# neuraloperator/graph-pde

Hardware: NVIDIA H100
Metric: NNConv edge-applications/s (higher is better)
Workload: dtype f16

## Files before the change

graph_pde_b200/csrc/api.cu:

```cuda
#include <cstdarg>
#include <cstdio>
#include <cstdlib>
#include <cstring>
#include <new>
#include <vector>

#include "common.cuh"
#include "kernels.h"
#include "options.h"

namespace nnc {

namespace {
thread_local char g_err[512] = "";
}

void set_error(const char* fmt, ...) {
  va_list ap;
  va_start(ap, fmt);
  vsnprintf(g_err, sizeof(g_err), fmt, ap);
  va_end(ap);
}

namespace {
// ... 315 lines not shown
  return launch_gemm_tc(W->prec, h, P->E, 0, static_cast<int>(P->E), W->Kp, W->W3n, NK, W->B3, 0, Kmat, NK, st, nullptr, 0, 0,
                        0, nullptr, nullptr, 0, 0, hpad);
}

int apply_edge(const Plan* P, const Weights* W, const void* Kmat, const float* x, const float* root, const float* bias,
               int aggr_mean, float* out, cudaStream_t st, unsigned node_flags) {
  NNC_REQUIRE(!(node_flags & NNCONV_APPLY_RESIDUAL) || W->cin == W->cout, NNCONV_ERR_ARG,
              "NNCONV_APPLY_RESIDUAL needs in_channels == out_channels");
  int s = launch_out_init(x, root, bias, P->N, W->cin, W->cout, out, st, node_flags);
  if (s) return s;
  if (P->E == 0 || P->n_src == 0) return NNCONV_OK;
  return launch_apply_edge(W->prec, P, W, Kmat, x, aggr_mean, out, st, node_flags);
}

struct ApplyLayout {
  size_t off_Xc, off_cvec, off_xs, off_flags, off_Y, fixed_bytes, per_node;
};
constexpr int kMaxPipeBatches = 1 << 14;

static ApplyLayout layout_apply(const Plan* P, const Weights* W) {
  Carver c(nullptr, ~size_t(0));
  ApplyLayout L{};
  const size_t S = P->n_src > 0 ? P->n_src : 1;
  L.off_Xc = c.off; c.take<char>((S + 128) * W->cin_p * W->esize * (W->split ? 3 : 1));
  L.off_cvec = c.off; c.take<float>(S * W->cout);
  L.off_xs = c.off; c.take<float>(S);
  L.off_flags = c.off; c.take<int>(5 * kMaxPipeBatches);
  L.off_Y = c.off;
  L.fixed_bytes = c.off;
  L.per_node = static_cast<size_t>(W->cout) * W->Kp * W->esize * (W->split ? 2 : 1);
  return L;
}

size_t apply_ws_bytes(const Plan* P, const Weights* W, size_t want_y_bytes) {
  ApplyLayout L = layout_apply(P, W);
  size_t nodes = want_y_bytes / L.per_node;
  if (nodes < 1) nodes = 1;
  if (nodes > static_cast<size_t>(P->n_src > 0 ? P->n_src : 1)) nodes = P->n_src > 0 ? P->n_src : 1;
  return L.fixed_bytes + nodes * L.per_node + 1024;
}

static bool fused_geometry(const Weights* W, int64_t n_src, int64_t nodes_cap, int* ring_out, int64_t* nb_out) {
  const Options& opt = options();
  const bool no_fuse_env = opt.no_fuse != 0 && !W->split;
  if (W->prec == PREC_FP32 || no_fuse_env || !apply_fused_supported(W)) return false;
  int ring = opt.ring;
  if (opt.ring_deep && nodes_cap / 128 > ring) ring = nodes_cap / 128 < 16 ? static_cast<int>(nodes_cap / 128) : 16;
  if (nodes_cap < ring) ring = nodes_cap >= 2 ? static_cast<int>(nodes_cap) : 1;
  int64_t nb = nodes_cap / ring;
  if (nb >= 128) nb = nb / 128 * 128;
  if (nb > n_src) nb = n_src;
  *ring_out = ring;
  *nb_out = nb;
  return ring >= 2;
}

int apply(const Plan* P, const Weights* W, const void* h, const float* x, const float* root, const float* bias,
          int aggr_mean, float* out, void* ws, size_t ws_bytes, cudaStream_t st, int64_t* launches, unsigned node_flags) {
  int s;
  NNC_REQUIRE(!(node_flags & NNCONV_APPLY_RESIDUAL) || W->cin == W->cout, NNCONV_ERR_ARG,
              "NNCONV_APPLY_RESIDUAL needs in_channels == out_channels");
  if (P->E == 0 || P->n_src == 0) {
    ProfScope ps(PK_NODE_PREP, st);
    s = launch_out_init(x, root, bias, P->N, W->cin, W->cout, out, st, node_flags);
    if (s == NNCONV_OK && launches) ++*launches;
    return s;
  }
  const bool tc = tc_shapes_supported(W);
// ... 103 lines not shown
  };
  auto launch_c = [&](int64_t b) -> int {
    const int64_t c0 = b * nb_max;
    const int nb = static_cast<int>((P->n_src - c0) < nb_max ? (P->n_src - c0) : nb_max);
    const int tb = h_tile_ptr[c0], te = h_tile_ptr[c0 + nb];
    PipeFlags pf{};
    pf.pdl = pipe;
    pf.wait_ok = pipe ? okY + b : nullptr;
    pf.done_cnt = pipe ? cntC + b : nullptr;
    pf.done_ok = pipe ? okC + b : nullptr;
    if (pipe && b == n_batches - 1) {
      pf.join_ok = okC;
      pf.join_n = static_cast<int>(n_batches - 1);
    }
    ProfScope ps(PK_CONV, st);
    return launch_conv_tc(W->prec, P, h, W->Kp, Ybuf[b % 3], nb, W->cout, tb, te, static_cast<int>(c0), cvec, xs,
                          aggr_mean, out, st, pipe ? &pf : nullptr);
  };
  s = launch_y(0);
  if (s) return s;
  for (int64_t b = 0; b < n_batches; ++b) {
    if (b + 1 < n_batches) {
      s = launch_y(b + 1);
      if (s) return s;
    }
    s = launch_c(b);
    if (s) return s;
  }
  if (launches) *launches += 2 * n_batches;
  return NNCONV_OK;
}

constexpr int64_t kUnitEdges = 2 * kTileEdges;
constexpr size_t kStreamYBytes = size_t(48) << 20;

static size_t h_row_bytes(const Weights* W) { return static_cast<size_t>(W->Kp) * 2 * (W->split ? 2 : 1); }

static int src_of_edge(const Plan* P, int64_t e) {
  const int* g = P->h_group_ptr;
  int lo = 0, hi = P->n_src;
  while (hi - lo > 1) {
    const int mid = (lo + hi) / 2;
    if (g[mid] <= e) lo = mid; else hi = mid;
  }
  return lo;
}

static int64_t unit_floor(const Plan* P, int64_t lim) {
  if (lim >= P->E) return P->E;
  if (lim <= 0) return 0;
  const int c = src_of_edge(P, lim);
  const int64_t g = P->h_group_ptr[c];
  return g + (lim - g) / kUnitEdges * kUnitEdges;
}

bool is_unit_boundary(const Plan* P, int64_t e) { return e >= 0 && e <= P->E && unit_floor(P, e) == e; }

static UnitRange edge_range(const Plan* P, int64_t e_lo, int64_t e_hi) {
  UnitRange r;
  const int c_lo = src_of_edge(P, e_lo);
  r.u_begin = P->h_unit_ptr[c_lo] + static_cast<int>((e_lo - P->h_group_ptr[c_lo]) / kUnitEdges);
  if (e_hi >= P->E) {
    r.u_end = P->n_units;
  } else {
    const int c_hi = src_of_edge(P, e_hi);
    r.u_end = P->h_unit_ptr[c_hi] + static_cast<int>((e_hi - P->h_group_ptr[c_hi]) / kUnitEdges);
  }
  r.c_begin = c_lo;
  r.c_end = src_of_edge(P, e_hi - 1) + 1;
  r.e_base = e_lo;
  r.h_rows = round_up64(e_hi - e_lo, 128);
  return r;
}

static int tile_at(const Plan* P, int64_t e) {
  if (e >= P->E) return P->n_tiles;
  const int c = src_of_edge(P, e);
  return P->h_tile_ptr[c] + static_cast<int>((e - P->h_group_ptr[c]) / kTileEdges);
}

struct StreamLayout {
  size_t off_apply, apply_bytes, off_h, off_ef, ef_bytes;
  int64_t rows;
};

static StreamLayout layout_stream(const Plan* P, const Weights* W, size_t ws_bytes) {
  StreamLayout L{};
  L.off_apply = kEfHeader;
  L.apply_bytes = round_up64(static_cast<int64_t>(apply_ws_bytes(P, W, kStreamYBytes)), 1024);
  L.off_h = L.off_apply + L.apply_bytes;
  const size_t fixed = L.off_h + 4096;
  const size_t row = h_row_bytes(W) + ef_row_bytes(W);
  L.rows = ws_bytes > fixed ? static_cast<int64_t>((ws_bytes - fixed) / row / 128 * 128) : 0;
  L.off_ef = L.off_h + static_cast<size_t>(L.rows) * h_row_bytes(W);
  L.ef_bytes = static_cast<size_t>(L.rows) * ef_row_bytes(W) + 4096;
  return L;
}

static int64_t count_chunks(const Plan* P, int64_t E_res, int64_t rows) {
  int64_t n = 0;
  for (int64_t e = E_res; e < P->E; e = unit_floor(P, e + rows)) ++n;
  return n;
}

int stream_split(const Plan* P, const Weights* W, size_t resident_bytes, size_t chunk_ws_bytes, int64_t* E_res,
                 size_t* h_res_bytes, size_t* ws_bytes, int64_t* n_chunks) {
  NNC_REQUIRE(W->prec == PREC_F16 || W->prec == PREC_BF16 || W->prec == PREC_F16X2, NNCONV_ERR_UNSUPPORTED,
              "streamed edge features need precision f16, bf16 or f16x2");
  const size_t hrow = h_row_bytes(W);
  const size_t full = static_cast<size_t>(round_up64(P->E, 128)) * hrow;
  *E_res = resident_bytes >= full ? P->E : unit_floor(P, static_cast<int64_t>(resident_bytes / hrow) / 128 * 128);
  *h_res_bytes = static_cast<size_t>(round_up64(*E_res, 128)) * hrow;
  const size_t row = hrow + ef_row_bytes(W);
  int64_t rows = static_cast<int64_t>(chunk_ws_bytes / row) / 128 * 128;
  const int64_t rest = round_up64(P->E - *E_res, 128);
  if (rows > rest) rows = rest;
  if (rows < kUnitEdges) rows = kUnitEdges;
  StreamLayout L = layout_stream(P, W, 0);
  *ws_bytes = L.off_h + 4096 + static_cast<size_t>(rows) * row;
  *n_chunks = count_chunks(P, *E_res, rows);
  return NNCONV_OK;
}
// ... 599 lines not shown
```

graph_pde_b200/csrc/apply_tc.cu:

```cuda
#include <type_traits>

#include "kernels.h"
#include "options.h"
#include "tc05.cuh"
#include "tmap.h"

namespace nnc {

int tc_num_sms();

namespace {

using namespace tc05;

constexpr int kMaxSlots = 16;
constexpr int kMaxAStages = 10;
constexpr int kTU = 2;
constexpr int kATileBytes = 128 * 64 * 2;
constexpr int kYStages = 2;
constexpr int kThreads = 14 * 32;
constexpr int kConvProducer = 12, kYProducer = 13;
constexpr int kQueue = 8;
constexpr int kScatterPitch = 272;
constexpr int kScatterBytes = 8 * 32 * kScatterPitch;
constexpr int kYScratchBytes = 4 * acc_scratch_bytes<16>();

struct ApplyArgs {
  const int* tile_c;
  const int* tile_e0;
  const int* tile_cnt;
  const int* tile_ptr;
  const int* unit_ptr;
  const int* unit_t;
  const int* unit_u;
  const int* dst_sorted;
  const float* inv_deg;
  const float* cvec;
  const float* xs;
  float* out;
  int u_begin, u_end, c_begin, c_end, e_base;
  int nb, n_batches, ring;
  int nb_slots, passes, a_stages, e_pad;
  int split_nk;
  int Kp;
  const float* y_scale;
  int NY;
  int num_kx;
  void* Yring;
  int* cntY;
  int* okY;
  int* cntC;
  int* okC;
  int* cntU;
  unsigned long long y_store_policy;
  unsigned long long a_policy;
  int scatter_mode;
  int debug_scatter;
  TraceBuf trace;
};

struct HMaps {
  CUtensorMap m[8];
};

__device__ __forceinline__ void raise_when_all(int* cnt, int* ok, int target) {
  const int prev = atomicAdd(cnt, 1);
  if (prev == target - 1) {
    __threadfence();
    asm volatile("st.release.gpu.global.s32 [%0], %1;" ::"l"(ok), "r"(1) : "memory");
  }
}

template <int FMT, int kYBlockN, int NC>
__global__ void __launch_bounds__(kThreads, 1)
k_apply_tc(const __grid_constant__ HMaps tmH, const __grid_constant__ CUtensorMap tmY,
           const __grid_constant__ CUtensorMap tmX, const __grid_constant__ CUtensorMap tmW, ApplyArgs a) {
  constexpr int kYStageBytes = kATileBytes + kYBlockN * 64 * 2;
  extern __shared__ __align__(1024) uint8_t smem[];
  if ((smem_u32(smem) & 1023u) != 0) __trap();
  const int b_chunk_bytes = NC * 128;
  const int b_stride = (b_chunk_bytes + 1023) & ~1023;
  uint8_t* smem_b = smem;
  uint8_t* smem_a = smem_b + a.nb_slots * b_stride;
  uint8_t* smem_y = smem_a + a.a_stages * kATileBytes;
  uint64_t* bars = reinterpret_cast<uint64_t*>(smem_y + kYStages * kYStageBytes);
  uint64_t* a_full = bars;
  uint64_t* a_empty = a_full + kMaxAStages;
  uint64_t* b_full = a_empty + kMaxAStages;
  uint64_t* b_empty = b_full + kMaxSlots;
  uint64_t* y_full = b_empty + kMaxSlots;
  uint64_t* y_empty = y_full + kYStages;
  uint64_t* q_full = y_empty + kYStages;
  uint64_t* q_empty = q_full + kQueue;
  int4* q_ent = reinterpret_cast<int4*>(q_empty + kQueue);
  float* y_scratch = reinterpret_cast<float*>(reinterpret_cast<uint8_t*>(bars) + 1024);
  uint8_t* smem_sc = reinterpret_cast<uint8_t*>(bars) + 1024 + kYScratchBytes;

  const int warp = __shfl_sync(0xffffffffu, static_cast<int>(threadIdx.x / 32), 0), lane = threadIdx.x % 32;
  const unsigned long long tr0 = a.trace.rec ? gtime() : 0ull;

  if (warp == kConvProducer && lane == 0) {
    for (int i = 0; i < 8; ++i) prefetch_tmap(&tmH.m[i]);
    prefetch_tmap(&tmY);
    prefetch_tmap(&tmX);
    prefetch_tmap(&tmW);
    for (int s = 0; s < a.a_stages; ++s) {
      mbar_init(&a_full[s], 1);
      mbar_init(&a_empty[s], 4);
    }
    for (int j = 0; j < a.nb_slots; ++j) {
      mbar_init(&b_full[j], 1);
      mbar_init(&b_empty[j], 8);
    }
    for (int s = 0; s < kYStages; ++s) {
      mbar_init(&y_full[s], 1);
      mbar_init(&y_empty[s], 4);
    }
    for (int s = 0; s < kQueue; ++s) {
      mbar_init(&q_full[s], 1);
      mbar_init(&q_empty[s], 8);
    }
    fence_barrier_init();
  }
  __syncthreads();

  if (warp == kConvProducer) {
    ARing ring[kTU];
#pragma unroll
    for (int ti = 0; ti < kTU; ++ti) ring[ti].init(ti, a.a_stages);
    int bs = 0;
    uint32_t bph = 0;
    const int num_kc = a.passes * a.nb_slots;
    int qi = 0;
    uint32_t qph = 0;
    auto publish = [&](int t, int u, int c, int b) {
      mbar_wait(&q_empty[qi], qph ^ 1u);
      if (elect_one()) {
        q_ent[qi] = make_int4(t, u, c, b);
        mbar_arrive(&q_full[qi]);
      }
      __syncwarp();
      if (++qi == kQueue) { qi = 0; qph ^= 1u; }
    };
    auto grab = [&]() {
      int v = 0;
      if (lane == 0) v = a.u_begin + atomicAdd(a.cntU, 1);
      return __shfl_sync(0xffffffffu, v, 0);
    };
    const int n_units = a.u_end;
    int nxt = grab();
    int cur_b = -1;
    while (nxt < n_units) {
      const int ui = nxt;
      nxt = grab();
// ... 32 lines not shown
        }
        __syncwarp();
        if (++bs == a.nb_slots) { bs = 0; bph ^= 1u; }
#pragma unroll
        for (int ti = 0; ti < kTU; ++ti) {
          if (ti < uu) {
            const CUtensorMap* mh = &tmH.m[tbox[ti] - 1];
            const uint32_t a_bytes = static_cast<uint32_t>(tbox[ti]) * 16u * 128u;
            const int stage = ring[ti].stage;
            mbar_wait(&a_empty[stage], ring[ti].phase ^ 1u);
            if (elect_one()) {
              mbar_arrive_expect_tx(&a_full[stage], a_bytes);
              tma_load_2d(smem_a + stage * kATileBytes, mh, &a_full[stage], 0, ja * a.e_pad + te0[ti] - a.e_base,
                          a.a_policy);
            }
            __syncwarp();
            ring[ti].next();
          }
        }
      }
    }
    publish(0, -1, 0, 0);
  } else if (warp < 8) {
    const int g = warp / 4, quarter = warp % 4;
    Acc<NC> acc;
    ARing ring;
    ring.init(g, a.a_stages);
    int bs = 0;
    uint32_t bph = 0;
    const int num_kc = a.passes * a.nb_slots;
    int qi = 0;
    uint32_t qph = 0;
    const int fr = lane >> 2, fc = (lane & 3) * 2;
    const uint32_t my_rows = smem_u32(smem_sc) + static_cast<uint32_t>(warp * 32 * kScatterPitch);
    for (;;) {
      mbar_wait(&q_full[qi], qph);
      int4 en = q_ent[qi];
      en.y = __shfl_sync(0xffffffffu, en.y, 0);
      __syncwarp();
      if (lane == 0) mbar_arrive(&q_empty[qi]);
      if (++qi == kQueue) { qi = 0; qph ^= 1u; }
      if (en.y < 0) break;
      if (en.y == 0) continue;
      for (int j = 0; j < num_kc; ++j) {
        mbar_wait(&b_full[bs], bph);
        const uint64_t bdesc = smem_desc_sw128(smem_u32(smem_b + bs * b_stride));
        if (g < en.y) {
          mbar_wait(&a_full[ring.stage], ring.phase);
          const uint64_t adesc = smem_desc_sw128(smem_u32(smem_a + ring.stage * kATileBytes));
          mma_block<NC, FMT>(acc, adesc, bdesc, 512, 2, 4, j != 0);
          wgmma_wait<0>();
          __syncwarp();
          if (lane == 0) mbar_arrive(&a_empty[ring.stage]);
          ring.next();
        }
        __syncwarp();
        if (lane == 0) mbar_arrive(&b_empty[bs]);
        if (++bs == a.nb_slots) { bs = 0; bph ^= 1u; }
      }
      named_bar_sync(1, 256);
      if (warp == 0 && lane == 0) {
        const int c0 = a.c_begin + en.w * a.nb;
        const int target = min(__ldg(a.unit_ptr + min(c0 + a.nb, a.c_end)), a.u_end) - max(__ldg(a.unit_ptr + c0), a.u_begin);
        raise_when_all(a.cntC + en.w, a.okC + en.w, target);
      }
      if (g >= en.y) continue;
      const int r = acc_row(quarter, lane);
      const bool ok = r < a.tile_cnt[en.x + g];
      int d = 0;
      float sc = 1.f;
      if (ok) {
        d = __ldg(a.dst_sorted + a.tile_e0[en.x + g] + r);
        if (a.inv_deg) sc = __ldg(a.inv_deg + d);
      }
      const float* cv = a.cvec + static_cast<int64_t>(en.z) * NC;
      const float xsc = __ldg(a.xs + en.z);
      float* orow = a.out + static_cast<int64_t>(d) * NC;
      int fd[4];
      float fsc[4];
      bool fok[4];
#pragma unroll
      for (int i = 0; i < 4; ++i) {
        const int L = fr + 8 * i;
        fd[i] = __shfl_sync(0xffffffffu, d, L);
        fsc[i] = __shfl_sync(0xffffffffu, sc, L);
        fok[i] = __shfl_sync(0xffffffffu, ok ? 1 : 0, L) != 0;
      }
      if (a.scatter_mode == 1) {
        bulk_wait_read0();
        __syncwarp();
#pragma unroll
        for (int jj = 0; jj < NC / 8; ++jj) {
          const float2 cq = __ldg(reinterpret_cast<const float2*>(cv + 8 * jj + fc));
#pragma unroll
          for (int i = 0; i < 4; ++i) {
            const float* dv = acc.d[i >> 1] + 4 * jj + 2 * (i & 1);
            const uint32_t addr = my_rows + static_cast<uint32_t>((fr + 8 * i) * kScatterPitch + (8 * jj + fc) * 4);
            asm volatile("st.shared.v2.f32 [%0], {%1, %2};" ::"r"(addr), "f"(fmaf(dv[0], xsc, cq.x) * fsc[i]),
                         "f"(fmaf(dv[1], xsc, cq.y) * fsc[i])
                         : "memory");
          }
        }
        fence_proxy_async_smem();
        __syncwarp();
        if (ok) bulk_reduce_add_f32(orow, my_rows + static_cast<uint32_t>(lane * kScatterPitch), static_cast<uint32_t>(NC) * 4u);
        bulk_commit();
      } else if (a.debug_scatter != 1) {
#pragma unroll
        for (int jj = 0; jj < NC / 8; ++jj) {
          const float2 cq = __ldg(reinterpret_cast<const float2*>(cv + 8 * jj + fc));
#pragma unroll
          for (int i = 0; i < 4; ++i) {
            if (!fok[i]) continue;
            const float* dv = acc.d[i >> 1] + 4 * jj + 2 * (i & 1);
            float* dst = a.out + static_cast<int64_t>(fd[i]) * NC + 8 * jj + fc;
            if (a.debug_scatter == 2) {
              *reinterpret_cast<float2*>(dst) = make_float2(dv[0], dv[1]);
            } else {
              asm volatile("red.global.add.v2.f32 [%0], {%1, %2};" ::"l"(dst), "f"(fmaf(dv[0], xsc, cq.x) * fsc[i]),
                           "f"(fmaf(dv[1], xsc, cq.y) * fsc[i])
                           : "memory");
            }
          }
        }
      }
    }
    if (a.scatter_mode == 1) bulk_wait0();
  } else if (warp == kYProducer) {
    const int n_blocks = a.NY / kYBlockN;
    int stage = 0;
    uint32_t phase = 0;
    for (int b = 0; b < a.n_batches; ++b) {
      const int c0 = a.c_begin + b * a.nb;
      const int rows = min(a.nb, a.c_end - c0);
      const int tiles = ((rows + 127) / 128) * n_blocks;
      for (int i = static_cast<int>((blockIdx.x + 7u * b) % gridDim.x); i < tiles; i += gridDim.x) {
        const int mb = i / n_blocks, nbk = i % n_blocks;
        for (int kx = 0; kx < a.num_kx; ++kx) {
          mbar_wait(&y_empty[stage], phase ^ 1u);
          if (elect_one()) {
            mbar_arrive_expect_tx(&y_full[stage], kYStageBytes);
            uint8_t* st = smem_y + stage * kYStageBytes;
            tma_load_2d(st, &tmX, &y_full[stage], kx * 64, c0 + mb * 128, kEvictLast);
            tma_load_2d(st + kATileBytes, &tmW, &y_full[stage], kx * 64, nbk * kYBlockN, kEvictLast);
          }
          __syncwarp();
          if (++stage == kYStages) { stage = 0; phase ^= 1u; }
        }
      }
    }
  } else {
    const int quarter = warp % 4;
    const int n_blocks = a.NY / kYBlockN;
    float* wb = y_scratch + quarter * (acc_scratch_bytes<16>() / 4);
    Acc<kYBlockN> acc;
    int stage = 0;
    uint32_t phase = 0;
    for (int b = 0; b < a.n_batches; ++b) {
      const int c0 = a.c_begin + b * a.nb;
      const int rows = min(a.nb, a.c_end - c0);
      const int tiles = ((rows + 127) / 128) * n_blocks;
      const unsigned long long ty0 = a.trace.rec ? gtime() : 0ull;
      if (b >= a.ring) {
        if (warp == 8 && lane == 0) flag_wait(a.okC + (b - a.ring), 500);
        named_bar_sync(2, 128);
      }
      const unsigned long long ty1 = a.trace.rec ? gtime() : 0ull;
      const int ymul = a.split_nk > 0 ? 2 : 1;
      const float ysc = a.y_scale != nullptr ? __ldg(a.y_scale) : 1.f;
      uint16_t* ybase = reinterpret_cast<uint16_t*>(a.Yring) + static_cast<int64_t>(b % a.ring) * a.nb * a.NY * ymul;
      for (int i = static_cast<int>((blockIdx.x + 7u * b) % gridDim.x); i < tiles; i += gridDim.x) {
        const int mb = i / n_blocks, nbk = i % n_blocks;
        for (int kx = 0; kx < a.num_kx; ++kx) {
          mbar_wait(&y_full[stage], phase);
          uint8_t* st = smem_y + stage * kYStageBytes;
          mma_block<kYBlockN, FMT>(acc, smem_desc_sw128(smem_u32(st)), smem_desc_sw128(smem_u32(st + kATileBytes)), 512, 2,
                                   4, kx != 0);
          wgmma_wait<0>();
          __syncwarp();
          if (lane == 0) mbar_arrive(&y_empty[stage]);
          if (++stage == kYStages) { stage = 0; phase ^= 1u; }
        }
        const int row = mb * 128 + acc_row(quarter, lane);
        const bool row_ok = row < rows;
        const int n0 = nbk * kYBlockN;
        uint16_t* yrow0 = ybase + static_cast<int64_t>(row) * a.NY * ymul;
#pragma unroll
        for (int cc = 0; cc < kYBlockN / 16; ++cc) {
          uint32_t vv[16];
          acc_rows<kYBlockN, 16>(acc, cc * 16, wb, vv);
          if (row_ok) {
            uint32_t packed[8], packed_lo[8];
#pragma unroll
            for (int j = 0; j < 8; ++j) {
              float f0 = __uint_as_float(vv[2 * j]), f1 = __uint_as_float(vv[2 * j + 1]);
              if (FMT == 0 && a.split_nk > 0) { f0 *= ysc; f1 *= ysc; }
              if (FMT == 0) {
                __half2 hh = __floats2half2_rn(f0, f1);
                packed[j] = *reinterpret_cast<uint32_t*>(&hh);
                if (a.split_nk > 0) {
                  const float2 hf = __half22float2(hh);
                  __half2 ll = __floats2half2_rn(f0 - hf.x, f1 - hf.y);
                  packed_lo[j] = *reinterpret_cast<uint32_t*>(&ll);
                }
              } else {
                __nv_bfloat162 hh = __floats2bfloat162_rn(f0, f1);
                packed[j] = *reinterpret_cast<uint32_t*>(&hh);
              }
            }
            const int n = n0 + cc * 16;
            uint16_t* yrow = yrow0 + n + (a.split_nk > 0 ? (n / a.Kp) * a.Kp : 0);
            st_global_32b_hint(yrow, packed, a.y_store_policy);
            if (FMT == 0 && a.split_nk > 0) st_global_32b_hint(yrow + a.Kp, packed_lo, a.y_store_policy);
          }
        }
      }
      __threadfence();
      __syncwarp();
      if (lane == 0) raise_when_all(a.cntY + b, a.okY + b, 4 * static_cast<int>(gridDim.x));
      if (a.trace.rec && warp == 8 && lane == 0 && (blockIdx.x % 37) == 0)
        trace_write(a.trace, 302u | (static_cast<unsigned>(b) << 12), ty0, ty1, gtime());
    }
  }
  __syncthreads();
  if (threadIdx.x == 0) trace_write(a.trace, 300u, tr0, tr0, a.trace.rec ? gtime() : 0ull);
}

struct ApplyShape {
  int nb_slots, passes, a_stages, smem_bytes;
};

bool apply_shape(int cout, int Kp, int ybn, ApplyShape* as) {
  const int kYStageBytes = kATileBytes + ybn * 64 * 2;
  if (cout % 16 != 0 || cout < 16 || cout > 64 || Kp % 64 != 0) return false;
  const int num_kc = Kp / 64;
  const int b_stride = (cout * 128 + 1023) & ~1023;
  const int bar_bytes = 1024 + kYScratchBytes + (options().scatter_mode == 1 ? kScatterBytes : 0);
  const int budget = 227 * 1024 - bar_bytes - kYStages * kYStageBytes;
  const int forced = options().apply_passes;
  for (int min_stages = 7; min_stages >= 3; min_stages -= 2) {
    for (int passes = 1; passes <= num_kc; ++passes) {
      if (num_kc % passes) continue;
      if (forced > 0 && passes != forced && num_kc % forced == 0) continue;
      const int nb = num_kc / passes;
      if (nb > kMaxSlots) continue;
      if (passes > 1 && nb < 4) continue;
      int stages = (budget - nb * b_stride) / kATileBytes;
      if (stages > kMaxAStages) stages = kMaxAStages;
      if (stages >= min_stages) {
        as->nb_slots = nb;
        as->passes = passes;
        as->a_stages = stages;
        as->smem_bytes = nb * b_stride + stages * kATileBytes + kYStages * kYStageBytes + bar_bytes;
        return true;
      }
    }
  }
  return false;
}

}

constexpr int kYBN = 64;

static int eff_kp(const Weights* W) { return W->split ? 3 * W->Kp : W->Kp; }

bool apply_fused_supported(const Weights* W) {
  if (W->prec != PREC_F16 && W->prec != PREC_BF16 && W->prec != PREC_F16X2) return false;
  if ((W->cout * W->Kp) % 128 != 0) return false;
  ApplyShape as;
  return apply_shape(W->cout, eff_kp(W), kYBN, &as);
}

namespace {
template <int FMT, int YBN, int NC>
int launch_variant(int grid, int smem_bytes, bool coop, cudaStream_t st, const HMaps& tmH, const CUtensorMap& tmY,
                   const CUtensorMap& tmX, const CUtensorMap& tmW, const ApplyArgs& a) {
  static bool attr_set = false;
  static int blocks_per_sm = -1;
  if (!attr_set) {
    NNC_CHECK_CUDA(cudaFuncSetAttribute(k_apply_tc<FMT, YBN, NC>, cudaFuncAttributeMaxDynamicSharedMemorySize, 227 * 1024));
    attr_set = true;
  }
  if (blocks_per_sm < 0)
    NNC_CHECK_CUDA(cudaOccupancyMaxActiveBlocksPerMultiprocessor(&blocks_per_sm, k_apply_tc<FMT, YBN, NC>, kThreads,
                                                                 smem_bytes));
  NNC_REQUIRE(blocks_per_sm >= 1, NNCONV_ERR_UNSUPPORTED, "apply_tc: the persistent kernel does not fit one SM");
  cudaLaunchConfig_t cfg{};
  cfg.gridDim = dim3(grid);
  cfg.blockDim = dim3(kThreads);
  cfg.dynamicSmemBytes = smem_bytes;
  cfg.stream = st;
  cudaLaunchAttribute attr[1];
  attr[0].id = cudaLaunchAttributeCooperative;
  attr[0].val.cooperative = 1;
  cfg.attrs = attr;
  cfg.numAttrs = coop ? 1 : 0;
  cudaError_t e = cudaLaunchKernelEx(&cfg, k_apply_tc<FMT, YBN, NC>, tmH, tmY, tmX, tmW, a);
  if (e == cudaErrorCooperativeLaunchTooLarge) {
    cudaGetLastError();
    return kApplyCannotCoSchedule;
  }
  NNC_CHECK_CUDA(e);
  return NNCONV_OK;
}
}

int launch_apply_tc(int prec, const Plan* P, const Weights* W, const void* h, const void* Xc, void* Yring, int nb,
                    int ring, const float* cvec, const float* xs, int aggr_mean, float* out, int* flags,
                    int flags_stride, cudaStream_t st, const UnitRange* range) {
  int s = tc_init();
  if (s != NNCONV_OK) return s;
  const Options& opt = options();
  const int bf = prec == PREC_BF16;
  const int split = W->split ? 1 : 0;
  const int ybn = kYBN;
  ApplyShape as;
  NNC_REQUIRE(apply_shape(W->cout, eff_kp(W), ybn, &as), NNCONV_ERR_UNSUPPORTED, "apply_tc: unsupported shape");
  if (opt.apply_stages >= 2 && opt.apply_stages < as.a_stages) as.a_stages = opt.apply_stages;
  const UnitRange whole{0, P->n_units, 0, P->n_src, 0, round_up64(P->E, 128)};
  const UnitRange& R = range ? *range : whole;
  const int64_t e_pad = R.h_rows;
  const int NY = W->cout * W->Kp;
  const int kmul = split ? 2 : 1;
  const int xmul = split ? 3 : 1;
  const int n_batches = ceil_div(R.c_end - R.c_begin, nb);
  NNC_REQUIRE(n_batches <= flags_stride, NNCONV_ERR_WORKSPACE, "apply_tc: too many source batches (%d)", n_batches);
  NNC_REQUIRE(static_cast<uint64_t>(kmul * W->Kp / 64) * e_pad < (1ull << 31), NNCONV_ERR_UNSUPPORTED,
              "apply_tc: edge-feature tensor exceeds 2^31 rows of 64 columns");
  HMaps tmH;
  CUtensorMap tmY, tmX, tmW;
  for (int i = 0; i < 8; ++i) {
    s = make_tmap_2d_16b(&tmH.m[i], bf, h, static_cast<uint64_t>(kmul * W->Kp / 64) * e_pad, 64, 16 * (i + 1));
    if (s != NNCONV_OK) return s;
  }
  s = make_tmap_2d_16b(&tmY, bf, Yring, static_cast<uint64_t>(ring) * nb * W->cout, static_cast<uint64_t>(kmul) * W->Kp,
                       W->cout);
  if (s != NNCONV_OK) return s;
  s = make_tmap_2d_16b(&tmX, bf, Xc, static_cast<uint64_t>(P->n_src), static_cast<uint64_t>(xmul) * W->cin_p, 128);
  if (s != NNCONV_OK) return s;
  s = make_tmap_2d_16b(&tmW, bf, W->W3p, static_cast<uint64_t>(NY), static_cast<uint64_t>(xmul) * W->cin_p, ybn);
  if (s != NNCONV_OK) return s;
  ApplyArgs a;
  a.tile_c = P->tile_c; a.tile_e0 = P->tile_e0; a.tile_cnt = P->tile_cnt; a.tile_ptr = P->tile_ptr;
  a.unit_ptr = P->unit_ptr; a.unit_t = P->unit_t; a.unit_u = P->unit_u;
  a.dst_sorted = P->dst_sorted; a.inv_deg = aggr_mean ? P->inv_deg : nullptr; a.cvec = cvec; a.xs = xs; a.out = out;
  a.u_begin = R.u_begin; a.u_end = R.u_end; a.c_begin = R.c_begin; a.c_end = R.c_end;
  a.e_base = static_cast<int>(R.e_base);
  a.nb = nb; a.n_batches = n_batches; a.ring = ring;
  a.nb_slots = as.nb_slots; a.passes = as.passes; a.a_stages = as.a_stages;
  a.e_pad = static_cast<int>(e_pad);
  a.split_nk = split ? W->Kp / 64 : 0;
  a.Kp = W->Kp;
  a.y_scale = (split && W->wscale) ? W->wscale + 2 * W->n_layers + 1 : nullptr;
  a.NY = NY; a.num_kx = xmul * W->cin_p / 64; a.Yring = Yring;
  a.y_store_policy = opt.y_store_policy == 1 ? kEvictLast : opt.y_store_policy == 2 ? kEvictFirst : kEvictNormal;
  a.a_policy = opt.apply_a_policy == 1 ? kEvictNormal : kEvictFirst;
  a.scatter_mode = (opt.scatter_mode == 1 && W->cout <= 64) ? 1 : 0;
  a.debug_scatter = opt.debug_scatter;
  a.cntY = flags; a.cntC = flags + flags_stride; a.okY = flags + 2 * flags_stride; a.okC = flags + 3 * flags_stride;
  a.cntU = flags + 4 * flags_stride;
  {
    TraceHandle th = trace_get();
    a.trace = TraceBuf{th.rec, th.count, th.cap};
  }
  bool window_set = false;
  if (opt.l2_persist > 0) {
    static int max_persist = -1;
    if (max_persist < 0) {
      int dev = 0;
      cudaGetDevice(&dev);
      cudaDeviceGetAttribute(&max_persist, cudaDevAttrMaxPersistingL2CacheSize, dev);
      if (opt.l2_persist > 1 && (static_cast<size_t>(opt.l2_persist) << 20) < static_cast<size_t>(max_persist))
        max_persist = opt.l2_persist << 20;
      if (max_persist > 0) cudaDeviceSetLimit(cudaLimitPersistingL2CacheSize, static_cast<size_t>(max_persist));
    }
    const size_t ring_bytes = static_cast<size_t>(ring) * nb * NY * 2 * kmul;
    if (max_persist > 0) {
      cudaStreamAttrValue v{};
      v.accessPolicyWindow.base_ptr = Yring;
      v.accessPolicyWindow.num_bytes = ring_bytes;
      v.accessPolicyWindow.hitRatio = ring_bytes <= static_cast<size_t>(max_persist)
                                          ? 1.0f
// ... 31 lines not shown
```

graph_pde_b200/nn_conv.py:

```python
import collections
import ctypes
import math
import os
import weakref

import torch
from torch.nn import Parameter

from . import _lib

__all__ = ['NNConv_old', 'NNConv', 'ECConv', 'stats', 'clear_caches', 'default_precision']

stats = {'launches': 0, 'plans_built': 0, 'edge_feature_passes': 0, 'applies': 0, 'weight_preps': 0,
         'streamed_chunk_passes': 0}

_PLAN_CACHE = collections.OrderedDict()
_PLAN_CACHE_MAX = int(os.environ.get('NNCONV_B200_PLAN_CACHE', '64'))
_PLAN_CACHE_MAX_BYTES = int(os.environ.get('NNCONV_B200_PLAN_CACHE_BYTES', str(2 << 30)))
_OVERFLOW_CHECK = os.environ.get('NNCONV_B200_OVERFLOW_CHECK', '1') != '0'
_Y_BYTES = int(os.environ.get('NNCONV_B200_Y_BYTES', str(48 << 20)))
_EF_WS_BYTES = int(os.environ.get('NNCONV_B200_EF_WS_BYTES', str(2 << 30)))
_BWD_WS_BYTES = int(os.environ.get('NNCONV_B200_BWD_WS_BYTES', str(2 << 30)))
_BWD_APPLY_WS_BYTES = int(os.environ.get('NNCONV_B200_BWD_APPLY_WS_BYTES', str(4 << 30)))
_BWD_MLP_WS_BYTES = int(os.environ.get('NNCONV_B200_BWD_MLP_WS_BYTES', str(4 << 30)))
_BWD_MODE = os.environ.get('NNCONV_B200_BACKWARD', 'auto')
_KEEP_ACTS_MAX_BYTES = int(os.environ.get('NNCONV_B200_KEEP_ACTS_BYTES', str(8 << 30)))
_EDGE_KERNELS = os.environ.get('NNCONV_B200_EDGE_KERNELS', 'auto')
_EDGE_KERNELS_MAX_DEG = 8
_EDGE_KERNELS_MAX_EDGES = int(os.environ.get('NNCONV_B200_EDGE_KERNELS_MAX_EDGES', '8192'))
_EDGE_KERNELS_MAX_BYTES = 2 << 30
_EDGE_FEATURE_BYTES = os.environ.get('NNCONV_B200_EDGE_FEATURE_BYTES')
_STREAM_MARGIN_BYTES = 1 << 30


def default_precision():
    return os.environ.get('NNCONV_B200_PRECISION', 'f16')


def clear_caches():
    _PLAN_CACHE.clear()


def _stream_ptr(device):
    return ctypes.c_void_p(torch.cuda.current_stream(device).cuda_stream)


def _ptr(t):
    return ctypes.c_void_p(t.data_ptr()) if t is not None else ctypes.c_void_p(0)


def _require_cuda(t, name):
    if not t.is_cuda:
        raise RuntimeError('graph_pde_b200.NNConv: `%s` must be a CUDA tensor (there is no CPU path); got %s'
# ... 642 lines not shown
```

Before: 505.2 million.

## Size Y ring from L2, keep X tile resident, stage Y stores via smem

Y workspace size now defaults to the part of the device L2 left after the output buffer and a headroom fraction, replacing the fixed 48 MB, so the Y ring is meant to stay L2-resident. The apply kernel can keep the X row-tile resident in shared memory across N-blocks instead of reloading it every stage. Y epilogue stores go through a swizzled shared-memory staging buffer so the global writes are coalesced 16-byte vector stores. Scatter buffers are halved by processing rows in two passes, and tiles are assigned to CTAs as contiguous ranges rather than strided, which improves X reuse. These changes add shared-memory pressure and complexity, and a smaller Y ring may mean more batches.

```diff
diff --git a/graph_pde_b200/csrc/api.cu b/graph_pde_b200/csrc/api.cu
--- a/graph_pde_b200/csrc/api.cu
+++ b/graph_pde_b200/csrc/api.cu
@@ -371,8 +371,31 @@
   return L;
 }
 
+constexpr int kL2HeadroomDiv = 8;
+
+static size_t default_y_bytes(const Plan* P, const Weights* W) {
+  static int l2_bytes[64] = {};
+  int dev = 0;
+  if (cudaGetDevice(&dev) != cudaSuccess || dev < 0 || dev >= 64) {
+    cudaGetLastError();
+    dev = 0;
+  }
+  if (l2_bytes[dev] <= 0 && cudaDeviceGetAttribute(&l2_bytes[dev], cudaDevAttrL2CacheSize, dev) != cudaSuccess) {
+    cudaGetLastError();
+    l2_bytes[dev] = 0;
+  }
+  const size_t l2 = static_cast<size_t>(l2_bytes[dev] > 0 ? l2_bytes[dev] : 50 << 20);
+  const size_t per_node = layout_apply(P, W).per_node;
+  const size_t used = static_cast<size_t>(P->N) * W->cout * sizeof(float) + l2 / kL2HeadroomDiv;
+  const size_t fit = l2 > used ? l2 - used : 0;
+  size_t floor_bytes = static_cast<size_t>(options().ring) * 128 * per_node;
+  if (floor_bytes > l2) floor_bytes = l2;
+  return fit > floor_bytes ? fit : floor_bytes;
+}
+
 size_t apply_ws_bytes(const Plan* P, const Weights* W, size_t want_y_bytes) {
   ApplyLayout L = layout_apply(P, W);
+  if (want_y_bytes == 0) want_y_bytes = default_y_bytes(P, W);
   size_t nodes = want_y_bytes / L.per_node;
   if (nodes < 1) nodes = 1;
   if (nodes > static_cast<size_t>(P->n_src > 0 ? P->n_src : 1)) nodes = P->n_src > 0 ? P->n_src : 1;
@@ -542,7 +565,6 @@
 }
 
 constexpr int64_t kUnitEdges = 2 * kTileEdges;
-constexpr size_t kStreamYBytes = size_t(48) << 20;
 
 static size_t h_row_bytes(const Weights* W) { return static_cast<size_t>(W->Kp) * 2 * (W->split ? 2 : 1); }
 
@@ -597,7 +619,7 @@
 static StreamLayout layout_stream(const Plan* P, const Weights* W, size_t ws_bytes) {
   StreamLayout L{};
   L.off_apply = kEfHeader;
-  L.apply_bytes = round_up64(static_cast<int64_t>(apply_ws_bytes(P, W, kStreamYBytes)), 1024);
+  L.apply_bytes = round_up64(static_cast<int64_t>(apply_ws_bytes(P, W, 0)), 1024);
   L.off_h = L.off_apply + L.apply_bytes;
   const size_t fixed = L.off_h + 4096;
   const size_t row = h_row_bytes(W) + ef_row_bytes(W);
diff --git a/graph_pde_b200/csrc/apply_tc.cu b/graph_pde_b200/csrc/apply_tc.cu
--- a/graph_pde_b200/csrc/apply_tc.cu
+++ b/graph_pde_b200/csrc/apply_tc.cu
@@ -22,8 +22,10 @@
 constexpr int kConvProducer = 12, kYProducer = 13;
 constexpr int kQueue = 8;
 constexpr int kScatterPitch = 272;
-constexpr int kScatterBytes = 8 * 32 * kScatterPitch;
-constexpr int kYScratchBytes = 4 * acc_scratch_bytes<16>();
+constexpr int kScatterRows = 16;
+constexpr int kScatterBytes = 8 * kScatterRows * kScatterPitch;
+constexpr int kMaxXBytes = 3 * kATileBytes;
+constexpr int kYStagingBytes = 4 * 32 * 128;
 
 struct ApplyArgs {
   const int* tile_c;
@@ -41,6 +43,8 @@
   int u_begin, u_end, c_begin, c_end, e_base;
   int nb, n_batches, ring;
   int nb_slots, passes, a_stages, e_pad;
+  int x_resident;
+  int y_bytes;
   int split_nk;
   int Kp;
   const float* y_scale;
@@ -75,15 +79,17 @@
 __global__ void __launch_bounds__(kThreads, 1)
 k_apply_tc(const __grid_constant__ HMaps tmH, const __grid_constant__ CUtensorMap tmY,
            const __grid_constant__ CUtensorMap tmX, const __grid_constant__ CUtensorMap tmW, ApplyArgs a) {
-  constexpr int kYStageBytes = kATileBytes + kYBlockN * 64 * 2;
+  constexpr int kWBytes = kYBlockN * 64 * 2;
   extern __shared__ __align__(1024) uint8_t smem[];
   if ((smem_u32(smem) & 1023u) != 0) __trap();
   const int b_chunk_bytes = NC * 128;
   const int b_stride = (b_chunk_bytes + 1023) & ~1023;
   uint8_t* smem_b = smem;
   uint8_t* smem_a = smem_b + a.nb_slots * b_stride;
-  uint8_t* smem_y = smem_a + a.a_stages * kATileBytes;
-  uint64_t* bars = reinterpret_cast<uint64_t*>(smem_y + kYStages * kYStageBytes);
+  const int y_stage_bytes = a.x_resident ? kWBytes : kATileBytes + kWBytes;
+  uint8_t* smem_x = smem_a + a.a_stages * kATileBytes;
+  uint8_t* smem_y = smem_x + (a.x_resident ? a.num_kx * kATileBytes : 0);
+  uint64_t* bars = reinterpret_cast<uint64_t*>(smem_a + a.a_stages * kATileBytes + a.y_bytes);
   uint64_t* a_full = bars;
   uint64_t* a_empty = a_full + kMaxAStages;
   uint64_t* b_full = a_empty + kMaxAStages;
@@ -92,9 +98,11 @@
   uint64_t* y_empty = y_full + kYStages;
   uint64_t* q_full = y_empty + kYStages;
   uint64_t* q_empty = q_full + kQueue;
-  int4* q_ent = reinterpret_cast<int4*>(q_empty + kQueue);
-  float* y_scratch = reinterpret_cast<float*>(reinterpret_cast<uint8_t*>(bars) + 1024);
-  uint8_t* smem_sc = reinterpret_cast<uint8_t*>(bars) + 1024 + kYScratchBytes;
+  uint64_t* x_full = q_empty + kQueue;
+  uint64_t* x_empty = x_full + 1;
+  int4* q_ent = reinterpret_cast<int4*>(x_empty + 1);
+  uint8_t* y_staging = reinterpret_cast<uint8_t*>(bars) + 1024;
+  uint8_t* smem_sc = reinterpret_cast<uint8_t*>(bars) + 1024 + kYStagingBytes;
 
   const int warp = __shfl_sync(0xffffffffu, static_cast<int>(threadIdx.x / 32), 0), lane = threadIdx.x % 32;
   const unsigned long long tr0 = a.trace.rec ? gtime() : 0ull;
@@ -120,6 +128,8 @@
       mbar_init(&q_full[s], 1);
       mbar_init(&q_empty[s], 8);
     }
+    mbar_init(x_full, 1);
+    mbar_init(x_empty, 4);
     fence_barrier_init();
   }
   __syncthreads();
@@ -218,7 +228,7 @@
     int qi = 0;
     uint32_t qph = 0;
     const int fr = lane >> 2, fc = (lane & 3) * 2;
-    const uint32_t my_rows = smem_u32(smem_sc) + static_cast<uint32_t>(warp * 32 * kScatterPitch);
+    const uint32_t my_rows = smem_u32(smem_sc) + static_cast<uint32_t>(warp * kScatterRows * kScatterPitch);
     for (;;) {
       mbar_wait(&q_full[qi], qph);
       int4 en = q_ent[qi];
@@ -273,24 +283,28 @@
         fok[i] = __shfl_sync(0xffffffffu, ok ? 1 : 0, L) != 0;
       }
       if (a.scatter_mode == 1) {
-        bulk_wait_read0();
-        __syncwarp();
-#pragma unroll
-        for (int jj = 0; jj < NC / 8; ++jj) {
-          const float2 cq = __ldg(reinterpret_cast<const float2*>(cv + 8 * jj + fc));
-#pragma unroll
-          for (int i = 0; i < 4; ++i) {
-            const float* dv = acc.d[i >> 1] + 4 * jj + 2 * (i & 1);
-            const uint32_t addr = my_rows + static_cast<uint32_t>((fr + 8 * i) * kScatterPitch + (8 * jj + fc) * 4);
-            asm volatile("st.shared.v2.f32 [%0], {%1, %2};" ::"r"(addr), "f"(fmaf(dv[0], xsc, cq.x) * fsc[i]),
-                         "f"(fmaf(dv[1], xsc, cq.y) * fsc[i])
-                         : "memory");
-          }
-        }
-        fence_proxy_async_smem();
-        __syncwarp();
-        if (ok) bulk_reduce_add_f32(orow, my_rows + static_cast<uint32_t>(lane * kScatterPitch), static_cast<uint32_t>(NC) * 4u);
-        bulk_commit();
+#pragma unroll
+        for (int h = 0; h < 2; ++h) {
+          bulk_wait_read0();
+          __syncwarp();
+#pragma unroll
+          for (int jj = 0; jj < NC / 8; ++jj) {
+            const float2 cq = __ldg(reinterpret_cast<const float2*>(cv + 8 * jj + fc));
+#pragma unroll
+            for (int i = 2 * h; i < 2 * h + 2; ++i) {
+              const float* dv = acc.d[i >> 1] + 4 * jj + 2 * (i & 1);
+              const uint32_t addr = my_rows + static_cast<uint32_t>((fr + 8 * (i & 1)) * kScatterPitch + (8 * jj + fc) * 4);
+              asm volatile("st.shared.v2.f32 [%0], {%1, %2};" ::"r"(addr), "f"(fmaf(dv[0], xsc, cq.x) * fsc[i]),
+                           "f"(fmaf(dv[1], xsc, cq.y) * fsc[i])
+                           : "memory");
+            }
+          }
+          fence_proxy_async_smem();
+          __syncwarp();
+          if (ok && (lane >> 4) == h)
+            bulk_reduce_add_f32(orow, my_rows + static_cast<uint32_t>((lane & 15) * kScatterPitch), static_cast<uint32_t>(NC) * 4u);
+          bulk_commit();
+        }
       } else if (a.debug_scatter != 1) {
 #pragma unroll
         for (int jj = 0; jj < NC / 8; ++jj) {
@@ -316,19 +330,35 @@
     const int n_blocks = a.NY / kYBlockN;
     int stage = 0;
     uint32_t phase = 0;
+    uint32_t xph = 0;
+    int x_b = -1, x_mb = -1;
     for (int b = 0; b < a.n_batches; ++b) {
       const int c0 = a.c_begin + b * a.nb;
       const int rows = min(a.nb, a.c_end - c0);
       const int tiles = ((rows + 127) / 128) * n_blocks;
-      for (int i = static_cast<int>((blockIdx.x + 7u * b) % gridDim.x); i < tiles; i += gridDim.x) {
+      const int64_t rot = (blockIdx.x + 7u * b) % gridDim.x;
+      const int t_end = static_cast<int>(tiles * (rot + 1) / gridDim.x);
+      for (int i = static_cast<int>(tiles * rot / gridDim.x); i < t_end; ++i) {
         const int mb = i / n_blocks, nbk = i % n_blocks;
+        if (a.x_resident && (b != x_b || mb != x_mb)) {
+          mbar_wait(x_empty, xph ^ 1u);
+          if (elect_one()) {
+            mbar_arrive_expect_tx(x_full, a.num_kx * kATileBytes);
+            for (int kx = 0; kx < a.num_kx; ++kx)
+              tma_load_2d(smem_x + kx * kATileBytes, &tmX, x_full, kx * 64, c0 + mb * 128, kEvictLast);
+          }
+          __syncwarp();
+          xph ^= 1u;
+          x_b = b;
+          x_mb = mb;
+        }
         for (int kx = 0; kx < a.num_kx; ++kx) {
           mbar_wait(&y_empty[stage], phase ^ 1u);
           if (elect_one()) {
-            mbar_arrive_expect_tx(&y_full[stage], kYStageBytes);
-            uint8_t* st = smem_y + stage * kYStageBytes;
-            tma_load_2d(st, &tmX, &y_full[stage], kx * 64, c0 + mb * 128, kEvictLast);
-            tma_load_2d(st + kATileBytes, &tmW, &y_full[stage], kx * 64, nbk * kYBlockN, kEvictLast);
+            mbar_arrive_expect_tx(&y_full[stage], y_stage_bytes);
+            uint8_t* st = smem_y + stage * y_stage_bytes;
+            if (!a.x_resident) tma_load_2d(st + kWBytes, &tmX, &y_full[stage], kx * 64, c0 + mb * 128, kEvictLast);
+            tma_load_2d(st, &tmW, &y_full[stage], kx * 64, nbk * kYBlockN, kEvictLast);
           }
           __syncwarp();
           if (++stage == kYStages) { stage = 0; phase ^= 1u; }
@@ -338,10 +368,13 @@
   } else {
     const int quarter = warp % 4;
     const int n_blocks = a.NY / kYBlockN;
-    float* wb = y_scratch + quarter * (acc_scratch_bytes<16>() / 4);
+    const uint32_t stg = smem_u32(y_staging) + static_cast<uint32_t>(quarter * 32 * 128);
+    const int fr = lane >> 2, fc = (lane & 3) * 2;
     Acc<kYBlockN> acc;
     int stage = 0;
     uint32_t phase = 0;
+    uint32_t xph = 0;
+    int x_b = -1, x_mb = -1;
     for (int b = 0; b < a.n_batches; ++b) {
       const int c0 = a.c_begin + b * a.nb;
       const int rows = min(a.nb, a.c_end - c0);
@@ -355,49 +388,80 @@
       const int ymul = a.split_nk > 0 ? 2 : 1;
       const float ysc = a.y_scale != nullptr ? __ldg(a.y_scale) : 1.f;
       uint16_t* ybase = reinterpret_cast<uint16_t*>(a.Yring) + static_cast<int64_t>(b % a.ring) * a.nb * a.NY * ymul;
-      for (int i = static_cast<int>((blockIdx.x + 7u * b) % gridDim.x); i < tiles; i += gridDim.x) {
+      const int64_t rot = (blockIdx.x + 7u * b) % gridDim.x;
+      const int t_end = static_cast<int>(tiles * (rot + 1) / gridDim.x);
+      for (int i = static_cast<int>(tiles * rot / gridDim.x); i < t_end; ++i) {
         const int mb = i / n_blocks, nbk = i % n_blocks;
+        if (a.x_resident && (b != x_b || mb != x_mb)) {
+          if (x_b >= 0) {
+            __syncwarp();
+            if (lane == 0) mbar_arrive(x_empty);
+          }
+          mbar_wait(x_full, xph);
+          xph ^= 1u;
+          x_b = b;
+          x_mb = mb;
+        }
         for (int kx = 0; kx < a.num_kx; ++kx) {
           mbar_wait(&y_full[stage], phase);
-          uint8_t* st = smem_y + stage * kYStageBytes;
-          mma_block<kYBlockN, FMT>(acc, smem_desc_sw128(smem_u32(st)), smem_desc_sw128(smem_u32(st + kATileBytes)), 512, 2,
-                                   4, kx != 0);
+          uint8_t* st = smem_y + stage * y_stage_bytes;
+          const uint8_t* xt = a.x_resident ? smem_x + kx * kATileBytes : st + kWBytes;
+          mma_block<kYBlockN, FMT>(acc, smem_desc_sw128(smem_u32(xt)), smem_desc_sw128(smem_u32(st)), 512, 2, 4, kx != 0);
           wgmma_wait<0>();
           __syncwarp();
           if (lane == 0) mbar_arrive(&y_empty[stage]);
           if (++stage == kYStages) { stage = 0; phase ^= 1u; }
         }
-        const int row = mb * 128 + acc_row(quarter, lane);
-        const bool row_ok = row < rows;
         const int n0 = nbk * kYBlockN;
-        uint16_t* yrow0 = ybase + static_cast<int64_t>(row) * a.NY * ymul;
-#pragma unroll
-        for (int cc = 0; cc < kYBlockN / 16; ++cc) {
-          uint32_t vv[16];
-          acc_rows<kYBlockN, 16>(acc, cc * 16, wb, vv);
-          if (row_ok) {
-            uint32_t packed[8], packed_lo[8];
-#pragma unroll
-            for (int j = 0; j < 8; ++j) {
-              float f0 = __uint_as_float(vv[2 * j]), f1 = __uint_as_float(vv[2 * j + 1]);
-              if (FMT == 0 && a.split_nk > 0) { f0 *= ysc; f1 *= ysc; }
+        const int ncol = n0 + (a.split_nk > 0 ? (n0 / a.Kp) * a.Kp : 0);
+        const int n_parts = (FMT == 0 && a.split_nk > 0) ? 2 : 1;
+        if (FMT == 0 && a.split_nk > 0) {
+#pragma unroll
+          for (int h = 0; h < 2; ++h)
+#pragma unroll
+            for (int k = 0; k < kYBlockN / 2; ++k) acc.d[h][k] *= ysc;
+        }
+#pragma unroll 1
+        for (int part = 0; part < n_parts; ++part) {
+          __syncwarp();
+#pragma unroll
+          for (int j = 0; j < kYBlockN / 8; ++j) {
+#pragma unroll
+            for (int q = 0; q < 4; ++q) {
+              const int R = 16 * (q >> 1) + fr + 8 * (q & 1);
+              float f0 = acc.d[q >> 1][4 * j + 2 * (q & 1)], f1 = acc.d[q >> 1][4 * j + 2 * (q & 1) + 1];
+              uint32_t p;
               if (FMT == 0) {
                 __half2 hh = __floats2half2_rn(f0, f1);
-                packed[j] = *reinterpret_cast<uint32_t*>(&hh);
-                if (a.split_nk > 0) {
+                if (part == 1) {
                   const float2 hf = __half22float2(hh);
-                  __half2 ll = __floats2half2_rn(f0 - hf.x, f1 - hf.y);
-                  packed_lo[j] = *reinterpret_cast<uint32_t*>(&ll);
+                  hh = __floats2half2_rn(f0 - hf.x, f1 - hf.y);
                 }
+                p = *reinterpret_cast<uint32_t*>(&hh);
               } else {
                 __nv_bfloat162 hh = __floats2bfloat162_rn(f0, f1);
-                packed[j] = *reinterpret_cast<uint32_t*>(&hh);
+                p = *reinterpret_cast<uint32_t*>(&hh);
               }
+              const uint32_t addr = stg + static_cast<uint32_t>(R * 128 + ((j ^ (R & 7)) << 4) + fc * 2);
+              asm volatile("st.shared.b32 [%0], %1;" ::"r"(addr), "r"(p) : "memory");
             }
-            const int n = n0 + cc * 16;
-            uint16_t* yrow = yrow0 + n + (a.split_nk > 0 ? (n / a.Kp) * a.Kp : 0);
-            st_global_32b_hint(yrow, packed, a.y_store_policy);
-            if (FMT == 0 && a.split_nk > 0) st_global_32b_hint(yrow + a.Kp, packed_lo, a.y_store_policy);
+          }
+          __syncwarp();
+          uint16_t* ytile = ybase + ncol + part * a.Kp;
+#pragma unroll
+          for (int it = 0; it < 8; ++it) {
+            const int R = 4 * it + (lane >> 3), ch = lane & 7;
+            const int row = mb * 128 + acc_row(quarter, R);
+            uint32_t v[4];
+            const uint32_t addr = stg + static_cast<uint32_t>(R * 128 + ((ch ^ (R & 7)) << 4));
+            asm volatile("ld.shared.v4.b32 {%0, %1, %2, %3}, [%4];" : "=r"(v[0]), "=r"(v[1]), "=r"(v[2]), "=r"(v[3]) : "r"(addr)
+                         : "memory");
+            if (row < rows) {
+              uint16_t* dst = ytile + static_cast<int64_t>(row) * a.NY * ymul + ch * 8;
+              asm volatile("st.global.L2::cache_hint.v4.b32 [%0], {%1, %2, %3, %4}, %5;" ::"l"(dst), "r"(v[0]), "r"(v[1]),
+                           "r"(v[2]), "r"(v[3]), "l"(a.y_store_policy)
+                           : "memory");
+            }
           }
         }
       }
@@ -413,32 +477,37 @@
 }
 
 struct ApplyShape {
-  int nb_slots, passes, a_stages, smem_bytes;
+  int nb_slots, passes, a_stages, x_resident, y_bytes, smem_bytes;
 };
 
-bool apply_shape(int cout, int Kp, int ybn, ApplyShape* as) {
-  const int kYStageBytes = kATileBytes + ybn * 64 * 2;
+bool apply_shape(int cout, int Kp, int ybn, int num_kx, ApplyShape* as) {
+  const int w_bytes = ybn * 64 * 2;
   if (cout % 16 != 0 || cout < 16 || cout > 64 || Kp % 64 != 0) return false;
   const int num_kc = Kp / 64;
   const int b_stride = (cout * 128 + 1023) & ~1023;
-  const int bar_bytes = 1024 + kYScratchBytes + (options().scatter_mode == 1 ? kScatterBytes : 0);
-  const int budget = 227 * 1024 - bar_bytes - kYStages * kYStageBytes;
+  const int bar_bytes = 1024 + kYStagingBytes + (options().scatter_mode == 1 ? kScatterBytes : 0);
   const int forced = options().apply_passes;
   for (int min_stages = 7; min_stages >= 3; min_stages -= 2) {
-    for (int passes = 1; passes <= num_kc; ++passes) {
-      if (num_kc % passes) continue;
-      if (forced > 0 && passes != forced && num_kc % forced == 0) continue;
-      const int nb = num_kc / passes;
-      if (nb > kMaxSlots) continue;
-      if (passes > 1 && nb < 4) continue;
-      int stages = (budget - nb * b_stride) / kATileBytes;
-      if (stages > kMaxAStages) stages = kMaxAStages;
-      if (stages >= min_stages) {
-        as->nb_slots = nb;
-        as->passes = passes;
-        as->a_stages = stages;
-        as->smem_bytes = nb * b_stride + stages * kATileBytes + kYStages * kYStageBytes + bar_bytes;
-        return true;
+    for (int xres = num_kx * kATileBytes <= kMaxXBytes ? 1 : 0; xres >= 0; --xres) {
+      const int y_bytes = xres ? num_kx * kATileBytes + kYStages * w_bytes : kYStages * (kATileBytes + w_bytes);
+      const int budget = 227 * 1024 - bar_bytes - y_bytes;
+      for (int passes = 1; passes <= num_kc; ++passes) {
+        if (num_kc % passes) continue;
+        if (forced > 0 && passes != forced && num_kc % forced == 0) continue;
+        const int nb = num_kc / passes;
+        if (nb > kMaxSlots) continue;
+        if (passes > 1 && nb < 4) continue;
+        int stages = (budget - nb * b_stride) / kATileBytes;
+        if (stages > kMaxAStages) stages = kMaxAStages;
+        if (stages >= min_stages) {
+          as->nb_slots = nb;
+          as->passes = passes;
+          as->a_stages = stages;
+          as->x_resident = xres;
+          as->y_bytes = y_bytes;
+          as->smem_bytes = nb * b_stride + stages * kATileBytes + y_bytes + bar_bytes;
+          return true;
+        }
       }
     }
   }
@@ -450,12 +519,13 @@
 constexpr int kYBN = 64;
 
 static int eff_kp(const Weights* W) { return W->split ? 3 * W->Kp : W->Kp; }
+static int y_num_kx(const Weights* W) { return (W->split ? 3 : 1) * W->cin_p / 64; }
 
 bool apply_fused_supported(const Weights* W) {
   if (W->prec != PREC_F16 && W->prec != PREC_BF16 && W->prec != PREC_F16X2) return false;
   if ((W->cout * W->Kp) % 128 != 0) return false;
   ApplyShape as;
-  return apply_shape(W->cout, eff_kp(W), kYBN, &as);
+  return apply_shape(W->cout, eff_kp(W), kYBN, y_num_kx(W), &as);
 }
 
 namespace {
@@ -502,7 +572,8 @@
   const int split = W->split ? 1 : 0;
   const int ybn = kYBN;
   ApplyShape as;
-  NNC_REQUIRE(apply_shape(W->cout, eff_kp(W), ybn, &as), NNCONV_ERR_UNSUPPORTED, "apply_tc: unsupported shape");
+  NNC_REQUIRE(apply_shape(W->cout, eff_kp(W), ybn, y_num_kx(W), &as), NNCONV_ERR_UNSUPPORTED,
+              "apply_tc: unsupported shape");
   if (opt.apply_stages >= 2 && opt.apply_stages < as.a_stages) as.a_stages = opt.apply_stages;
   const UnitRange whole{0, P->n_units, 0, P->n_src, 0, round_up64(P->E, 128)};
   const UnitRange& R = range ? *range : whole;
@@ -535,6 +606,7 @@
   a.e_base = static_cast<int>(R.e_base);
   a.nb = nb; a.n_batches = n_batches; a.ring = ring;
   a.nb_slots = as.nb_slots; a.passes = as.passes; a.a_stages = as.a_stages;
+  a.x_resident = as.x_resident; a.y_bytes = as.y_bytes;
   a.e_pad = static_cast<int>(e_pad);
   a.split_nk = split ? W->Kp / 64 : 0;
   a.Kp = W->Kp;
diff --git a/graph_pde_b200/nn_conv.py b/graph_pde_b200/nn_conv.py
--- a/graph_pde_b200/nn_conv.py
+++ b/graph_pde_b200/nn_conv.py
@@ -18,7 +18,7 @@
 _PLAN_CACHE_MAX = int(os.environ.get('NNCONV_B200_PLAN_CACHE', '64'))
 _PLAN_CACHE_MAX_BYTES = int(os.environ.get('NNCONV_B200_PLAN_CACHE_BYTES', str(2 << 30)))
 _OVERFLOW_CHECK = os.environ.get('NNCONV_B200_OVERFLOW_CHECK', '1') != '0'
-_Y_BYTES = int(os.environ.get('NNCONV_B200_Y_BYTES', str(48 << 20)))
+_Y_BYTES = int(os.environ.get('NNCONV_B200_Y_BYTES', '0'))
 _EF_WS_BYTES = int(os.environ.get('NNCONV_B200_EF_WS_BYTES', str(2 << 30)))
 _BWD_WS_BYTES = int(os.environ.get('NNCONV_B200_BWD_WS_BYTES', str(2 << 30)))
 _BWD_APPLY_WS_BYTES = int(os.environ.get('NNCONV_B200_BWD_APPLY_WS_BYTES', str(4 << 30)))
```

Result: faster. 532.9 million, median of 6 (+5.5%).
